# ooowedyn/InkLayer

Hardware: AMD Instinct MI355X
Metric: sketches/sec end-to-end (GroundingDINO+SAM) at 1024x1024 (higher is better)
Workload: dtype f16 (MFMA, f32 accumulate; f32 residual/norm/softmax; split-f16 = fp32-grade operands for patch-embed, neck, mask decoder); 1 GPU; full GroundingDINO Swin-T + SAM ViT-H pipeline, batch=8 per GPU, 1024x1024 synthetic sketches, 16 boxes/sketch, random-init weights; global_batch=8, parallelism=image-parallel x1

## Files before the change

### include/inklayer_hip.h

```cpp
#ifndef INKLAYER_HIP_H
#define INKLAYER_HIP_H

#include <stdint.h>

#ifdef __cplusplus
extern "C" {
#endif

#define INK_ABI_VERSION 10
int ink_abi_version(void);

typedef struct InkGemm {
  const void* A;
  const void* W;
  const float* bias;
  const float* col_scale;
  const float* residual;
  const int32_t* row_map;
  void* C;
  int32_t M, N, K;
  int32_t lda, ldw, ldr, ldc;
  int32_t act;
  int32_t c_f16;
} InkGemm;
// ... 17 lines not shown
int ink_add_f32(const float* a, const float* b, int64_t n_b, float* out, int64_t n, void* stream);

typedef struct InkAttn {
  const void* Q; const void* K; const void* V;
  void* O;
  int64_t ldq, ldk, ldv, ldo;
  int32_t n_batch, n_heads, n_q, n_k, head_dim;
  float scale;
  int32_t bias_mode;
  int32_t grid_w;
  const int32_t* q_batch_rows;
  const int32_t* kv_batch_rows;
  const float* rel_h; const float* rel_w;
  const void* rel_aug;
  const float* dense_bias; const float* dense_mask;
  int32_t n_mask; int32_t rel_f16;
  const int32_t* tok_rows;
  const void* pad_k; const void* pad_v;
} InkAttn;
int ink_flash_attn(const InkAttn* p, void* stream);

int ink_swin_attn(const void* Q, const void* K, const void* V, int64_t ldq, int64_t ldk, int64_t ldv,
                  void* O, int64_t ldo, int32_t n_windows, int32_t n_heads, int32_t ws, float scale,
                  const float* bias_table, const uint8_t* region, int32_t nW, void* stream);

int ink_relpos_bias64_f16(const void* Q, int64_t ldq, const float* rel_pos_h, const float* rel_pos_w, int32_t n_batch,
                          int32_t n_heads, int32_t head_dim, float scale, void* out_h_f16, void* out_w_f16, void* stream);

int ink_relpos_bias(const void* Q, int64_t ldq, const float* rel_pos_h, const float* rel_pos_w,
                    int32_t S, int32_t n_batch, int32_t n_heads, int32_t head_dim, float scale,
                    const int32_t* tok_rows, float* out_h, float* out_w, void* out_aug_f16,
                    void* stream);

int ink_sam_patchify(const void* image_u8, int32_t h, int32_t w, int32_t L, int32_t P,
                     const float* mean3, const float* std3, int32_t chan_reverse, int32_t split,
                     void* out_f16, void* stream);

int ink_resize_u8(const void* src_u8, int32_t h, int32_t w, int32_t channels, void* dst_u8, int32_t oh, int32_t ow,
                  const int32_t* xbounds, const int32_t* xcoef, int32_t kx, const int32_t* ybounds,
                  const int32_t* ycoef, int32_t ky, void* tmp_u8, void* stream);

int ink_im2col3x3_f16(const void* in_f16, int32_t B, int32_t H, int32_t W, int32_t C, int32_t stride, int32_t relu,
                      void* out_f16, void* stream);

int ink_sam_pe_encode(const float* coords01, const float* gauss, int32_t N, int32_t F,
                      const float* add, int32_t n_add, float* out, void* stream);

int ink_sam_prompt_tokens(const float* points, const int32_t* labels, int32_t n_pts, int32_t pad, const float* boxes,
                          const float* gauss, int32_t F, const float* point_emb, const float* not_a_point,
                          const float* out_tok, float input_size, int32_t P, float* out, void* stream);

int ink_sam_mask_embed(const float* mask, const float* emb, const int32_t* emb_rows, const float* params,
                       int32_t n_params, float eps, int32_t P, int32_t g, float* keys, void* split_f16, void* stream);

int ink_sam_mask_logits(const float* up, const float* hyper, int32_t n, int32_t g, int32_t C,
                        float* out, void* stream);

int ink_sam_postprocess(const float* low, int32_t n, int32_t S, int32_t L, int32_t in_h,
                        int32_t in_w, int32_t out_h, int32_t out_w, float thr, void* out_u8,
                        float* out_logits, void* stream);

int ink_ms_deform_attn_forward(const float* value, const int64_t* spatial_shapes_host,
                               const int64_t* level_start_index_host, const float* sampling_loc,
                               const float* attn_weight, int32_t B, int32_t S, int32_t M, int32_t C,
                               int32_t Q, int32_t L, int32_t P, int32_t im2col_step, float* out,
                               void* stream);
// ... 252 lines not shown
```

### inklayer_amd/_lib.py

```python
from __future__ import annotations

import ctypes as C
import os
from pathlib import Path

_LIB_PATH = Path(__file__).resolve().parent / "lib" / "libinklayer_hip.so"
_lib = None

c_void_p, c_int, c_i64, c_float = C.c_void_p, C.c_int32, C.c_int64, C.c_float


class InkGemm(C.Structure):
    _fields_ = [
        ("A", c_void_p), ("W", c_void_p), ("bias", c_void_p), ("col_scale", c_void_p),
        ("residual", c_void_p), ("row_map", c_void_p), ("C", c_void_p),
        ("M", c_int), ("N", c_int), ("K", c_int),
        ("lda", c_int), ("ldw", c_int), ("ldr", c_int), ("ldc", c_int),
        ("act", c_int), ("c_f16", c_int),
    ]


class InkAttn(C.Structure):
    _fields_ = [
        ("Q", c_void_p), ("K", c_void_p), ("V", c_void_p), ("O", c_void_p),
        ("ldq", c_i64), ("ldk", c_i64), ("ldv", c_i64), ("ldo", c_i64),
        ("n_batch", c_int), ("n_heads", c_int), ("n_q", c_int), ("n_k", c_int),
        ("head_dim", c_int), ("scale", c_float), ("bias_mode", c_int), ("grid_w", c_int),
        ("q_batch_rows", c_void_p), ("kv_batch_rows", c_void_p),
        ("rel_h", c_void_p), ("rel_w", c_void_p), ("rel_aug", c_void_p),
        ("dense_bias", c_void_p), ("dense_mask", c_void_p), ("n_mask", c_int), ("rel_f16", c_int),
        ("tok_rows", c_void_p), ("pad_k", c_void_p), ("pad_v", c_void_p),
    ]


SIGNATURES = {
    "ink_abi_version": [],
    "ink_gemm_f16": [C.POINTER(InkGemm), c_void_p],
    "ink_gemm_set_variant": [c_int],
    "ink_gemm_query_variant": [c_int, c_int, c_int],
    "ink_layernorm_rows": [c_void_p, c_i64, c_void_p, c_void_p, c_float, c_void_p, c_int, c_int,
                           c_void_p, c_void_p, c_i64, c_int, c_int, c_void_p, c_i64, c_void_p, c_int, c_void_p],
    "ink_add_split_f16": [c_void_p, c_void_p, c_i64, c_void_p, c_i64, c_int, c_void_p],
    "ink_add_cvt_f16": [c_void_p, c_void_p, c_i64, c_void_p, c_i64, c_void_p],
    "ink_add_f32": [c_void_p, c_void_p, c_i64, c_void_p, c_i64, c_void_p],
    "ink_flash_attn": [C.POINTER(InkAttn), c_void_p],
    "ink_swin_attn": [c_void_p, c_void_p, c_void_p, c_i64, c_i64, c_i64, c_void_p, c_i64, c_int, c_int, c_int, c_float,
                      c_void_p, c_void_p, c_int, c_void_p],
    "ink_sam_patchify": [c_void_p, c_int, c_int, c_int, c_int, C.POINTER(c_float), C.POINTER(c_float),
                         c_int, c_int, c_void_p, c_void_p],
    "ink_im2col3x3_f16": [c_void_p, c_int, c_int, c_int, c_int, c_int, c_int, c_void_p, c_void_p],
    "ink_resize_u8": [c_void_p, c_int, c_int, c_int, c_void_p, c_int, c_int, c_void_p, c_void_p, c_int,
                      c_void_p, c_void_p, c_int, c_void_p, c_void_p],
    "ink_sam_pe_encode": [c_void_p, c_void_p, c_int, c_int, c_void_p, c_int, c_void_p, c_void_p],
    "ink_sam_mask_logits": [c_void_p, c_void_p, c_int, c_int, c_int, c_void_p, c_void_p],
    "ink_sam_prompt_tokens": [c_void_p, c_void_p, c_int, c_int, c_void_p, c_void_p, c_int, c_void_p, c_void_p,
                              c_void_p, c_float, c_int, c_void_p, c_void_p],
    "ink_sam_mask_embed": [c_void_p, c_void_p, c_void_p, c_void_p, c_int, c_float, c_int, c_int, c_void_p, c_void_p,
                           c_void_p],
    "ink_sam_postprocess": [c_void_p, c_int, c_int, c_int, c_int, c_int, c_int, c_int, c_float,
                            c_void_p, c_void_p, c_void_p],
    "ink_sam_amg_stats": [c_void_p, c_int, c_void_p, c_int, c_void_p, c_int, c_int, c_int, c_int, c_int, c_int, C.c_double,
                          C.c_double, c_int, c_int, c_int, c_int, c_void_p, c_void_p, c_void_p, c_void_p],
    "ink_mask_rle_counts": [c_void_p, c_void_p, c_int, c_int, c_int, c_void_p, c_void_p],
    "ink_mask_rle_write": [c_void_p, c_void_p, c_int, c_int, c_int, c_void_p, c_void_p, c_void_p],
    "ink_mask_small_regions_workspace_ints": [c_int, c_int, c_int, C.POINTER(c_i64)],
    "ink_mask_small_regions": [c_void_p, c_int, c_int, c_int, c_int, c_int, c_void_p, c_void_p, c_void_p, c_void_p,
                               c_void_p],
    "ink_box_nms": [c_void_p, c_void_p, c_int, c_float, c_void_p, c_void_p, c_void_p, c_void_p],
    "ink_ms_deform_attn_forward": [c_void_p, C.POINTER(c_i64), C.POINTER(c_i64), c_void_p, c_void_p, c_int,
                                   c_int, c_int, c_int, c_int, c_int, c_int, c_int, c_void_p, c_void_p],
# ... 141 lines not shown
```

### inklayer_amd/csrc/gemm.hip

```cpp
#include <stdlib.h>

#include "mfma_util.h"
#include "../../include/inklayer_hip.h"

namespace {

template <int BK> struct Swz;
template <> struct Swz<64> {
  static __device__ __forceinline__ int f(int row) { return row & 7; }
};
template <> struct Swz<32> {
  static __device__ __forceinline__ int f(int row) { return (-(row >> 2)) & 3; }
};

__device__ __forceinline__ bool residual_preloaded(const InkGemm& p) {
  return p.residual && p.act == INK_ACT_NONE && !p.col_scale;
}

template <int TM>
__device__ __forceinline__ void wave_rows(int (&rows)[TM], const InkGemm& p, int mw, int lane) {
#pragma unroll
  for (int ti = 0; ti < TM; ++ti) {
    const int m = mw + ti * 16 + (lane & 15);
    int r = -1;
    if (m < p.M) r = p.row_map ? p.row_map[m] : m;
    rows[ti] = r;
  }
}

template <int TM, int TN>
__device__ __forceinline__ void init_wave_tile(f32x4 (&acc)[TM][TN], const InkGemm& p, const int (&rows)[TM], int nw,
                                               int lane) {
  const int fq = lane >> 4;
  const bool pre = residual_preloaded(p);
#pragma unroll
  for (int ti = 0; ti < TM; ++ti) {
    const int r = pre ? rows[ti] : -1;
    const float* rp = p.residual + (size_t)max(r, 0) * p.ldr + nw + fq * 4;
#pragma unroll
    for (int j = 0; j < TN; ++j) {
      acc[ti][j] = (f32x4){0.f, 0.f, 0.f, 0.f};
      if (r >= 0 && nw + j * 16 + fq * 4 < p.N) acc[ti][j] = *(const f32x4*)(rp + j * 16);
    }
  }
}

template <int TM, int TN>
__device__ __forceinline__ void add_bias_wave_tile(f32x4 (&acc)[TM][TN], const InkGemm& p, int nw, int lane) {
  const int fq = lane >> 4;
#pragma unroll
  for (int j = 0; j < TN; ++j) {
    const int n = nw + j * 16 + fq * 4;
    f32x4 bv = (f32x4){0.f, 0.f, 0.f, 0.f};
    if (p.bias && n < p.N) bv = *(const f32x4*)(p.bias + n);
#pragma unroll
    for (int ti = 0; ti < TM; ++ti) acc[ti][j] += bv;
  }
}

template <int TM, int TN, int OUT, int MODE = -1>
__device__ __forceinline__ void store_wave_tile(f32x4 (&acc)[TM][TN], const InkGemm& p, char* er,
                                                const int (&rows)[TM], int nw, int lane) {
  constexpr bool F16O = OUT == 1;
  constexpr int WNC = TN * 16, EP = WNC * 4 + 16;
  constexpr int ES = OUT == 0 ? 4 : 8;
  constexpr int CPRW = WNC / ES;
  constexpr int NIT = (16 * CPRW + 63) / 64;
  const int fr = lane & 15, fq = lane >> 4;
  const bool wide16 = OUT != 0 && (p.ldc % 8 == 0);
  const bool res_late = MODE < 0 && p.residual && !residual_preloaded(p);
  const int act = MODE < 0 ? p.act : MODE;
  const bool scaled = MODE < 0 && p.col_scale != nullptr;
  int row_of[NIT], n_of[NIT];
#pragma unroll
  for (int it = 0; it < NIT; ++it) {
    const int c = it * 64 + lane;
    row_of[it] = c < 16 * CPRW ? c / CPRW : 16;
    n_of[it] = nw + (c % CPRW) * ES;
  }

  add_bias_wave_tile<TM, TN>(acc, p, nw, lane);

#pragma unroll
  for (int ti = 0; ti < TM; ++ti) {
#pragma unroll
    for (int j = 0; j < TN; ++j) {
      f32x4 v = acc[ti][j];
      if (act == INK_ACT_GELU) {
#pragma unroll
        for (int r = 0; r < 4; ++r) v[r] = gelu_erf(v[r]);
      } else if (act == INK_ACT_RELU) {
#pragma unroll
        for (int r = 0; r < 4; ++r) v[r] = fmaxf(v[r], 0.f);
      }
      if (scaled) {
        const int n = nw + j * 16 + fq * 4;
        if (n < p.N) v *= *(const f32x4*)(p.col_scale + n);
      }
      if (F16O) {
        *(f16x4*)(er + fr * EP + (j * 16 + fq * 4) * 2) = (f16x4){(f16)v[0], (f16)v[1], (f16)v[2], (f16)v[3]};
      } else {
        *(f32x4*)(er + fr * EP + (j * 16 + fq * 4) * 4) = v;
      }
    }
#pragma unroll
    for (int it = 0; it < NIT; ++it) {
      int r = __builtin_amdgcn_ds_bpermute((row_of[it] & 15) << 2, rows[ti]);
      if (row_of[it] >= 16 || n_of[it] >= p.N) r = -1;
      if (r >= 0) {
        const int c_n = n_of[it];
        const char* src = er + row_of[it] * EP + (c_n - nw) * (F16O ? 2 : 4);
        if (F16O) {
          f16x8 d = *(const f16x8*)src;
          f16* dst = (f16*)p.C + (size_t)r * p.ldc + c_n;
          if (res_late) {
            const float* rp = p.residual + (size_t)r * p.ldr + c_n;
#pragma unroll
            for (int e = 0; e < 8; ++e)
              if (c_n + e < p.N) d[e] = (f16)((float)d[e] + rp[e]);
          }
          if (wide16 && c_n + 8 <= p.N) {
            *(f16x8*)dst = d;
          } else {
            *(f16x4*)dst = (f16x4){d[0], d[1], d[2], d[3]};
            if (c_n + 8 <= p.N) *(f16x4*)(dst + 4) = (f16x4){d[4], d[5], d[6], d[7]};
          }
        } else {
          f32x4 d = *(const f32x4*)src;
          if (res_late) d += *(const f32x4*)(p.residual + (size_t)r * p.ldr + c_n);
          *(f32x4*)((float*)p.C + (size_t)r * p.ldc + c_n) = d;
        }
      }
    }
  }
}

__device__ __forceinline__ void tile_of(int id, int ntm, int ntn, int group_m, int& mt, int& nt) {
  if (group_m > 1) {
    const int per = group_m * ntn;
    const int first = (id / per) * group_m;
    const int gsz = min(ntm - first, group_m);
    mt = first + (id % per) % gsz;
    nt = (id % per) / gsz;
  } else {
    mt = id / ntn;
    nt = id % ntn;
  }
}

constexpr int NS = 2;
template <int BM, int BN, int BK, int WM, int WN>
__global__ __launch_bounds__(WM * WN * 64) void gemm_f16_nt(InkGemm p, int group_m) {
  constexpr int NT = WM * WN * 64;
  constexpr int CPR = BK / 8;
  constexpr int ROWB = BK * 2;
  constexpr int TILE_A = BM * ROWB, TILE_W = BN * ROWB;
  constexpr int STAGE = TILE_A + TILE_W;
  constexpr int IT_A = (BM * CPR) / NT, IT_W = (BN * CPR) / NT;
  constexpr int TM = BM / WM / 16, TN = BN / WN / 16;
  static_assert((BM * CPR) % NT == 0 && (BN * CPR) % NT == 0, "tile/threads mismatch");
  extern __shared__ __attribute__((aligned(16))) char smem[];

  const int tid = threadIdx.x;
  const int lane = tid & 63;
  const int wave = tid >> 6;
  const int wm = wave / WN, wn = wave % WN;

// ... 58 lines not shown
      for (int i0 = 0; i0 < TM; i0 += AG) {
#pragma unroll
        for (int i = 0; i < AG; ++i) a[i] = *(const f16x8*)(bA + offA + (i0 + i) * 16 * ROWB + co);
#pragma unroll
        for (int i = 0; i < AG; ++i)
#pragma unroll
          for (int j = 0; j < TN; ++j)
            acc[i0 + i][j] = __builtin_amdgcn_mfma_f32_16x16x32_f16(w[j], a[i], acc[i0 + i][j], 0, 0, 0);
      }
    }
  };

  stage(0, 0);
  init_wave_tile<TM, TN>(acc, p, rows, n0 + wn * (BN / WN), lane);
  for (int kt = 0; kt < nk; ++kt) {
    asm volatile("s_waitcnt vmcnt(0)" ::: "memory");
    __syncthreads();
    if (kt + 1 < nk) stage((kt + 1) & 1, kt + 1);
    compute(kt & 1);
  }

  constexpr int WNC = BN / WN;
  constexpr int EP = WNC * 4 + 16;
  static_assert(WM * WN * 16 * EP <= NS * STAGE, "epilogue patch must fit in the staging LDS");
  __syncthreads();
  char* er = smem + wave * (16 * EP);
  if (p.c_f16 == 1) {
    store_wave_tile<TM, TN, 1>(acc, p, er, rows, n0 + wn * WNC, lane);
  } else {
    store_wave_tile<TM, TN, 0>(acc, p, er, rows, n0 + wn * WNC, lane);
  }
}

constexpr int PP_RING = 4, PP_TN = 5;
__global__ __launch_bounds__(512) void gemm_f16_nt_pp(InkGemm p, int group_m) {
  constexpr int RING = PP_RING, TN = PP_TN;
  constexpr int BM = 256, BN = 64 * TN, BK = 32, NT = 512;
  constexpr int CPR = BK / 8, ROWB = BK * 2;
  constexpr int TILE_A = BM * ROWB, TILE_W = BN * ROWB, GRAN = TILE_A + TILE_W;
  constexpr int IT_A = (BM * CPR) / NT, IT_W = (BN * CPR) / NT;
  constexpr bool W_TAIL = (BN * CPR) % NT != 0;
  static_assert(!W_TAIL || (BN * CPR) % NT == NT / 2, "tail is exactly the first four waves");
  constexpr int LOADS = IT_A + IT_W;
  constexpr int TM = 8, WNC = 16 * TN;
  constexpr int AHEAD = RING - 2;
  constexpr int AG = 4;
  constexpr int EP = WNC * 4 + 16;
  static_assert(8 * 16 * EP <= RING * GRAN, "patch fits");
  extern __shared__ __attribute__((aligned(16))) char smem[];
  const int tid = threadIdx.x, lane = tid & 63;
  const int wave = __builtin_amdgcn_readfirstlane(tid >> 6);
  const int grp = wave >> 2, wn = wave & 3;
  const int fr = lane & 15, fq = lane >> 4;

  const int ntn = (p.N + BN - 1) / BN, ntm = (p.M + BM - 1) / BM;
  int mt, nt;
  tile_of(xcd_remap(blockIdx.x, ntm * ntn), ntm, ntn, group_m, mt, nt);
  const int m0 = mt * BM, n0 = nt * BN;
  const int G = p.K / BK;
  const f16* __restrict__ A = (const f16*)p.A;
  const f16* __restrict__ W = (const f16*)p.W;
  const f16* srcA[IT_A];
  const f16* srcW[IT_W + (W_TAIL ? 1 : 0)];
#pragma unroll
  for (int it = 0; it < IT_A; ++it) {
    const int pch = it * NT + tid, row = pch / CPR, lch = (pch % CPR) ^ Swz<BK>::f(row);
    srcA[it] = A + (size_t)min(m0 + row, p.M - 1) * p.lda + lch * 8;
  }
#pragma unroll
  for (int it = 0; it < IT_W + (W_TAIL ? 1 : 0); ++it) {
    const int pch = it * NT + tid, row = min(pch / CPR, BN - 1), lch = (pch % CPR) ^ Swz<BK>::f(row);
    srcW[it] = W + (size_t)min(n0 + row, p.N - 1) * p.ldw + lch * 8;
  }
  auto dma = [&](int g, int slot) {
    char* base = smem + slot * GRAN;
#pragma unroll
    for (int it = 0; it < IT_A; ++it)
      __builtin_amdgcn_global_load_lds((gptr_t)(srcA[it] + g * BK), (lptr_t)(base + (it * NT + wave * 64) * 16), 16, 0, 0);
#pragma unroll
    for (int it = 0; it < IT_W; ++it)
      __builtin_amdgcn_global_load_lds((gptr_t)(srcW[it] + g * BK), (lptr_t)(base + TILE_A + (it * NT + wave * 64) * 16), 16, 0, 0);
    if (W_TAIL && grp == 0)
      __builtin_amdgcn_global_load_lds((gptr_t)(srcW[IT_W] + g * BK), (lptr_t)(base + TILE_A + (IT_W * NT + wave * 64) * 16), 16, 0, 0);
  };
  auto wait_ahead = [&]() {
    if (W_TAIL && grp == 0) {
      asm volatile("s_waitcnt vmcnt(%0)" ::"n"((AHEAD - 1) * (LOADS + 1)) : "memory");
    } else {
      asm volatile("s_waitcnt vmcnt(%0)" ::"n"((AHEAD - 1) * LOADS) : "memory");
    }
  };
  auto slot_end = [&]() {
    __builtin_amdgcn_sched_barrier(0);
    __builtin_amdgcn_s_barrier();
    __builtin_amdgcn_sched_barrier(0);
  };

  int rows[TM];
  wave_rows<TM>(rows, p, m0 + grp * 128, lane);
#pragma unroll
  for (int g = 0; g < AHEAD; ++g) dma(g, g);
  f32x4 acc[TM][TN];
  init_wave_tile<TM, TN>(acc, p, rows, n0 + wn * WNC, lane);
  if (residual_preloaded(p)) {
    asm volatile("s_waitcnt vmcnt(0)" ::: "memory");
  } else {
    wait_ahead();
  }
  slot_end();
  if (grp == 1) slot_end();

  const int offA = (grp * 128 + fr) * ROWB;
  const int offW = (wn * WNC + fr) * ROWB;
  const int co = (fq ^ Swz<BK>::f(fr)) << 4;
  f16x8 a[AG], w[TN];
  int cslot = 0, islot = AHEAD % RING;
  auto iter = [&](int g) __attribute__((always_inline)) {
    const char* bA = smem + cslot * GRAN;
    const char* bW = bA + TILE_A;
#pragma unroll
    for (int i = 0; i < AG; ++i) a[i] = *(const f16x8*)(bA + offA + i * 16 * ROWB + co);
#pragma unroll
    for (int j = 0; j < TN; ++j) w[j] = *(const f16x8*)(bW + offW + j * 16 * ROWB + co);
    if (g + AHEAD < G) {
      dma(g + AHEAD, islot);
      wait_ahead();
    } else {
      asm volatile("s_waitcnt vmcnt(0)" ::: "memory");
    }
    slot_end();
    asm volatile("s_waitcnt lgkmcnt(0)" ::: "memory");
    __builtin_amdgcn_sched_barrier(0);
    __builtin_amdgcn_s_setprio(1);
#pragma unroll
    for (int i0 = 0; i0 < TM; i0 += AG) {
#pragma unroll
      for (int i = 0; i < AG; ++i) {
#pragma unroll
        for (int j = 0; j < TN; ++j)
          acc[i0 + i][j] = __builtin_amdgcn_mfma_f32_16x16x32_f16(w[j], a[i], acc[i0 + i][j], 0, 0, 0);
        if (i0 + AG < TM) {
          a[i] = *(const f16x8*)(bA + offA + (i0 + AG + i) * 16 * ROWB + co);
          __builtin_amdgcn_sched_barrier(0);
        }
      }
    }
    __builtin_amdgcn_s_setprio(0);
    slot_end();
    cslot = (cslot + 1 == RING) ? 0 : cslot + 1;
    islot = (islot + 1 == RING) ? 0 : islot + 1;
  };
  for (int g = 0; g < G; ++g) iter(g);
  if (grp == 0) slot_end();

  char* er = smem + wave * (16 * EP);
  const bool plain = !p.col_scale && !(p.residual && !residual_preloaded(p));
  if (p.c_f16) {
    if (plain && p.act == INK_ACT_GELU) {
      store_wave_tile<TM, TN, 1, INK_ACT_GELU>(acc, p, er, rows, n0 + wn * WNC, lane);
    } else if (plain && p.act == INK_ACT_NONE) {
      store_wave_tile<TM, TN, 1, INK_ACT_NONE>(acc, p, er, rows, n0 + wn * WNC, lane);
    } else {
      store_wave_tile<TM, TN, 1>(acc, p, er, rows, n0 + wn * WNC, lane);
    }
  } else {
    if (plain && p.act == INK_ACT_NONE) {
      store_wave_tile<TM, TN, 0, INK_ACT_NONE>(acc, p, er, rows, n0 + wn * WNC, lane);
    } else {
      store_wave_tile<TM, TN, 0>(acc, p, er, rows, n0 + wn * WNC, lane);
    }
  }
}

static int launch_gemm_pp(const InkGemm& p, hipStream_t s, int group_m) {
  if (p.K / 32 < PP_RING) return INK_ERR_ARG;
  constexpr int BN = 64 * PP_TN;
  constexpr int lds = PP_RING * (256 + BN) * 32 * 2;
  static_assert(lds <= 160 * 1024, "LDS budget");
  ink_dyn_lds<gemm_f16_nt_pp>(lds);
  const int ntiles = ((p.M + 255) / 256) * ((p.N + BN - 1) / BN);
  hipLaunchKernelGGL(gemm_f16_nt_pp, dim3(ntiles), dim3(512), lds, s, p, group_m);
  return ink_launch_status();
}

template <int BM, int BN, int BK, int WM, int WN>
static int launch_gemm(const InkGemm& p, hipStream_t s, int group_m = 1) {
  constexpr int lds = NS * (BM + BN) * BK * 2;
  static_assert(lds <= 160 * 1024, "LDS budget");
  ink_dyn_lds<gemm_f16_nt<BM, BN, BK, WM, WN>>(lds);
  const int ntm = (p.M + BM - 1) / BM, ntn = (p.N + BN - 1) / BN;
  hipLaunchKernelGGL((gemm_f16_nt<BM, BN, BK, WM, WN>), dim3(ntm * ntn), dim3(WM * WN * 64), lds, s, p, group_m);
  return ink_launch_status();
}

struct ConvGeom {
  int H, W, C, OH, OW, stride;
};
__device__ __attribute__((aligned(128))) const uint32_t g_conv_zero_row[32] = {};

template <int BK, bool RELU_IN>
__global__ __launch_bounds__(256) void conv3x3_f16_nt(InkGemm p, ConvGeom g) {
  constexpr int BM = 128, BN = 128, WM = 2, WN = 2;
  constexpr int NT = WM * WN * 64;
  constexpr int CPR = BK / 8;
  constexpr int ROWB = BK * 2;
  constexpr int TILE_A = BM * ROWB, TILE_W = BN * ROWB;
  constexpr int STAGE = TILE_A + TILE_W;
  constexpr int IT_A = (BM * CPR) / NT, IT_W = (BN * CPR) / NT;
  constexpr int TM = BM / WM / 16, TN = BN / WN / 16;
  extern __shared__ __attribute__((aligned(16))) char smem[];

  const int tid = threadIdx.x;
  const int lane = tid & 63;
  const int wave = tid >> 6;
// ... 165 lines not shown
  const long tiles256 = (long)((M + 255) / 256) * ((N + 255) / 256);
  const bool n_fits = (N % 256 == 0) || N >= 1024;
  return (tiles256 >= 200 && n_fits) ? 10 : 0;
}
extern "C" int ink_abi_version(void) { return INK_ABI_VERSION; }
extern "C" int ink_gemm_set_variant(int32_t v) {
  INK_CHECK_ARG(v == -1 || v == 0 || v == 10 || v == 45);
  g_variant = v;
  return INK_OK;
}

extern "C" int ink_gemm_f16(const InkGemm* pp, void* stream) {
  INK_CHECK_ARG(pp != nullptr);
  const InkGemm& p = *pp;
  INK_CHECK_ARG(p.A && p.W && p.C);
  INK_CHECK_ARG(p.M > 0 && p.N > 0 && p.K > 0);
  INK_CHECK_ARG(p.K % 32 == 0 && p.N % 4 == 0);
  INK_CHECK_ARG(p.lda % 8 == 0 && p.ldw % 8 == 0 && p.lda >= p.K && p.ldw >= p.K);
  INK_CHECK_ARG(p.ldc % 4 == 0 && p.ldc >= p.N);
  INK_CHECK_ARG(!p.residual || (p.ldr % 4 == 0 && p.ldr >= p.N));
  INK_CHECK_ARG(ink_aligned<16>(p.A, p.W, p.C));
  INK_CHECK_ARG(p.act >= 0 && p.act <= 2);
  INK_CHECK_ARG(p.c_f16 == 0 || p.c_f16 == 1);
  hipStream_t s = (hipStream_t)stream;
  if (p.K % 64 != 0) return launch_gemm<128, 128, 32, 2, 2>(p, s);
  int v = g_variant;
  if (v < 0) v = ink_gemm_query_variant(p.M, p.N, p.K);
  switch (v) {
    case 10: return launch_gemm<256, 256, 64, 4, 4>(p, s, 4);
    case 45: return launch_gemm_pp(p, s, 4);
    default: return launch_gemm<128, 128, 64, 2, 2>(p, s);
  }
}
```

### inklayer_amd/ops.py

```python
from __future__ import annotations

import ctypes as C
from typing import Optional, Sequence, Tuple

import torch

from . import _lib
from ._lib import InkAttn, InkGemm, check

ACT = {None: 0, "none": 0, "gelu": 1, "relu": 2}
F16, F32 = torch.float16, torch.float32


_GEMM_TRACE = None


def set_gemm_trace(lst) -> None:
    global _GEMM_TRACE
    _GEMM_TRACE = lst


_ATTN_TRACE = None


def set_attn_trace(lst) -> None:
    global _ATTN_TRACE
    _ATTN_TRACE = lst


def tracing_off() -> bool:
    return _GEMM_TRACE is None and _ATTN_TRACE is None


_raw_stream = getattr(torch._C, "_cuda_getCurrentRawStream", None)
_cur_device = getattr(torch._C, "_cuda_getDevice", None)


def _stream() -> int:
    if _raw_stream is not None and _cur_device is not None:
        return _raw_stream(_cur_device())
    return torch.cuda.current_stream().cuda_stream


def own_f32(t: torch.Tensor, dev) -> torch.Tensor:
    t = t.detach().to(dev, F32).contiguous()
    if t.untyped_storage().nbytes() > t.numel() * t.element_size():
        t = t.clone()
    return t


def _p(t: Optional[torch.Tensor]) -> Optional[int]:
    if t is None:
        return None
    assert t.is_cuda, "InkLayer HIP ops need GPU tensors (no CPU fallback)"
    return t.data_ptr()


def gemm(a: torch.Tensor, w: torch.Tensor, bias: Optional[torch.Tensor] = None, *,
         act: Optional[str] = None, residual: Optional[torch.Tensor] = None,
         col_scale: Optional[torch.Tensor] = None, row_map: Optional[torch.Tensor] = None,
         out: Optional[torch.Tensor] = None, out_dtype: torch.dtype = F32,
         out_rows: Optional[int] = None) -> torch.Tensor:
    assert a.dtype == F16 and w.dtype == F16
    assert a.dim() == 2 and w.dim() == 2 and a.stride(1) == 1 and w.stride(1) == 1
    M, K = a.shape
    N = w.shape[0]
    assert w.shape[1] == K
    p = InkGemm()
    if out is None:
        rows = out_rows if out_rows is not None else M
        out = torch.empty((rows, N), device=a.device, dtype=out_dtype)
    assert out.dim() == 2 and out.stride(1) == 1 and out.shape[1] == N
    p.A, p.W, p.C = a.data_ptr(), w.data_ptr(), out.data_ptr()
    p.bias, p.col_scale = _p(bias), _p(col_scale)
    p.residual, p.row_map = _p(residual), _p(row_map)
    if bias is not None:
        assert bias.dtype == F32 and bias.numel() == N
    if col_scale is not None:
        assert col_scale.dtype == F32 and col_scale.numel() == N
    if residual is not None:
        assert residual.dtype == F32 and residual.stride(1) == 1 and residual.shape[1] == N
        p.ldr = residual.stride(0)
    if row_map is not None:
        assert row_map.dtype == torch.int32 and row_map.numel() == M
    p.M, p.N, p.K = M, N, K
    p.lda, p.ldw, p.ldc = a.stride(0), w.stride(0), out.stride(0)
    p.act = ACT[act]
    p.c_f16 = 1 if out.dtype == F16 else 0
    assert out.dtype in (F16, F32)
    if _GEMM_TRACE is None:
        check(_lib.lib().ink_gemm_f16(C.byref(p), _stream()), "ink_gemm_f16")
    else:
        e0, e1 = torch.cuda.Event(enable_timing=True), torch.cuda.Event(enable_timing=True)
        e0.record()
        check(_lib.lib().ink_gemm_f16(C.byref(p), _stream()), "ink_gemm_f16")
        e1.record()
        _GEMM_TRACE.append((2.0 * M * N * K, e0, e1, (M, N, K, act or '-', 'res' if residual is not None else '-',
                                                      'map' if row_map is not None else '-', 'f16' if p.c_f16 else 'f32')))
    return out


def layernorm_rows(x: torch.Tensor, gamma: Optional[torch.Tensor], beta: Optional[torch.Tensor],
                   eps: float, *, gather: Optional[torch.Tensor] = None,
                   out_dtype: torch.dtype = F16, out: Optional[torch.Tensor] = None,
                   out2: Optional[torch.Tensor] = None, act: Optional[str] = None,
                   split: bool = False, add: Optional[torch.Tensor] = None,
                   add_batch_rows: Optional[torch.Tensor] = None, rows_per_batch: int = 0,
                   split_f32: Optional[torch.Tensor] = None) -> torch.Tensor:
    assert x.dtype == F32 and x.dim() == 2 and x.stride(1) == 1
    Cdim = x.shape[1]
    rows = gather.numel() if gather is not None else x.shape[0]
    wcols = 3 * Cdim if split else Cdim
    if split:
        assert out_dtype == F16 and out2 is None
    if out is None:
        out = torch.empty((rows, wcols), device=x.device, dtype=out_dtype)
    assert out.shape == (rows, wcols) and out.stride(1) == 1
    oh = out.data_ptr() if out.dtype == F16 else None
    of = out.data_ptr() if out.dtype == F32 else None
    if out2 is not None:
        assert out2.shape == out.shape and out2.stride(0) == out.stride(0) and out2.dtype != out.dtype
        if out2.dtype == F16:
            oh = out2.data_ptr()
        else:
            of = out2.data_ptr()
    if split_f32 is not None:
        assert split and out.stride(0) == 3 * Cdim and split_f32.dtype == F32 and split_f32.is_contiguous()
        assert tuple(split_f32.shape) == (rows, Cdim)
# ... 1327 lines not shown
```

### inklayer_amd/sam.py

```python
from __future__ import annotations

import math
from dataclasses import dataclass, replace
from typing import Dict, List, Optional, Sequence, Tuple

import numpy as np
import torch

from . import ops
from ._lru import LRU

F16, F32 = torch.float16, torch.float32


@dataclass
class SamConfig:
    embed_dim: int = 1280
    depth: int = 32
    num_heads: int = 16
    global_attn_indexes: Tuple[int, ...] = (7, 15, 23, 31)
    window_size: int = 14
    img_size: int = 1024
    patch_size: int = 16
    mlp_ratio: float = 4.0
# ... 197 lines not shown
            "the fused decoder kernels (csrc/proj_ln.hip, csrc/upscale_tail.hip) are built for SAM's widths"
        self.scale = cfg.head_dim ** -0.5
        sd = state_dict
        dev = self.dev

        def h(name):
            return sd[name].detach().to(torch.float32).to(dev, F16).contiguous()

        def f(name):
            return ops.own_f32(sd[name], dev)

        def ws(name, shape=None):
            t = sd[name].detach().to(dev, torch.float32)
            return ops.split_weight(t if shape is None else shape(t))

        self.w: Dict[str, torch.Tensor] = {}
        w = self.w
        P = cfg.patch_size
        w["pe.ws"] = ws("image_encoder.patch_embed.proj.weight", lambda t: t.reshape(D, 3 * P * P))
        w["pe.b"] = f("image_encoder.patch_embed.proj.bias")
        w["pos"] = f("image_encoder.pos_embed").reshape(self.T, D).contiguous()
        for i in range(cfg.depth):
            p = f"image_encoder.blocks.{i}."
            for n in ("norm1.weight", "norm1.bias", "norm2.weight", "norm2.bias", "attn.qkv.bias",
                      "attn.proj.bias", "mlp.lin1.bias", "mlp.lin2.bias", "attn.rel_pos_h",
                      "attn.rel_pos_w"):
                w[f"b{i}.{n}"] = f(p + n)
            for n in ("attn.qkv.weight", "attn.proj.weight", "mlp.lin1.weight", "mlp.lin2.weight"):
                w[f"b{i}.{n}"] = h(p + n)
            if i not in cfg.global_attn_indexes:
                qb = w[f"b{i}.attn.qkv.bias"]
                w[f"b{i}.pad_k"] = qb[D:2 * D].to(F16).contiguous()
                w[f"b{i}.pad_v"] = qb[2 * D:].to(F16).contiguous()
        w["neck0.ws"] = ws("image_encoder.neck.0.weight", lambda t: t.reshape(E, D))
        w["neck1.w"], w["neck1.b"] = f("image_encoder.neck.1.weight"), f("image_encoder.neck.1.bias")
        w["neck2.ws"] = ws("image_encoder.neck.2.weight", lambda t: t.permute(0, 2, 3, 1).reshape(E, 9, E)) \
            .reshape(E, 27 * E).contiguous()
        w["neck3.w"], w["neck3.b"] = f("image_encoder.neck.3.weight"), f("image_encoder.neck.3.bias")

        w["gauss"] = f("prompt_encoder.pe_layer.positional_encoding_gaussian_matrix")
        w["no_mask"] = f("prompt_encoder.no_mask_embed.weight").reshape(-1).contiguous()
        w["pt_emb"] = torch.cat([f(f"prompt_encoder.point_embeddings.{i}.weight") for i in range(4)], 0).contiguous()
        if "prompt_encoder.not_a_point_embed.weight" in sd:
            w["not_a_point"] = f("prompt_encoder.not_a_point_embed.weight").reshape(-1).contiguous()
        md = "prompt_encoder.mask_downscaling."
        md_names = ("0.weight", "0.bias", "1.weight", "1.bias", "3.weight", "3.bias", "4.weight", "4.bias", "6.weight",
                    "6.bias")
        if all(md + n in sd for n in md_names):
            w["mask_ds"] = torch.cat([sd[md + n].detach().to(torch.float32).reshape(-1) for n in md_names]) \
                .to(dev).contiguous()
        ar = (torch.arange(g, dtype=torch.float32) + 0.5) / g
        grid_xy = torch.stack([ar[None, :].expand(g, g), ar[:, None].expand(g, g)], -1).reshape(-1, 2)
        self.dense_pe = ops.sam_pe_encode(grid_xy.contiguous().to(dev), w["gauss"])

        t = "mask_decoder.transformer."
        def attn(dst, src):
            for n in ("q_proj", "k_proj", "v_proj", "out_proj"):
                w[f"{dst}.{n}.ws"] = ws(f"{src}.{n}.weight")
                w[f"{dst}.{n}.b"] = f(f"{src}.{n}.bias")

        def cat(dst, names):
            for sfx in (".ws", ".b"):
                w[dst + sfx] = torch.cat([w[n + sfx] for n in names]).contiguous()

        pe_split = ops.add_split_f16(self.dense_pe)
        for i in range(cfg.dec_depth):
# ... 95 lines not shown
            ops.sam_patchify(img, cfg.img_size, cfg.patch_size, cfg.pixel_mean, cfg.pixel_std,
                             chan_reverse, self.buf_patches[b * T:(b + 1) * T], split=True)
        ops.gemm(self.buf_patches[:B * T], w["pe.ws"], w["pe.b"], residual=self.pos_rep[:B * T], out=x)
        if upto is None and self.graph_blocks and ops.tracing_off():
            return self._blocks_graphed(B)
        return self._blocks(B, upto)

    graph_blocks = False
    graph_cache_size = 2

    def _blocks_graphed(self, B: int) -> torch.Tensor:
        g = self._enc_graphs.get(B)
        if g is None:
            self._enc_seen[B] = self._enc_seen.get(B, 0) + 1
            if self._enc_seen[B] < 2:
                return self._blocks(B, None)
            x0 = self.x[:B * self.T].clone()
            cur = torch.cuda.current_stream(self.dev)
            side = torch.cuda.Stream(device=self.dev)
            side.wait_stream(cur)
            with torch.cuda.stream(side):
                self._blocks(B, None)
                self.x[:B * self.T].copy_(x0)
            cur.wait_stream(side)
            graph = torch.cuda.CUDAGraph()
            with torch.cuda.graph(graph):
                out = self._blocks(B, None)
            self.x[:B * self.T].copy_(x0)
            g = (graph, out)
            self._enc_graphs.put(B, g)
        g[0].replay()
        return g[1].clone()

    def _blocks(self, B: int, upto: Optional[int]) -> torch.Tensor:
        cfg, w, T, D = self.cfg, self.w, self.T, self.cfg.embed_dim
        H, Mw = cfg.num_heads, self.Mw
        x = self.x[:B * T]
        nblk = cfg.depth if upto is None else upto
        calib = getattr(self, "_calib", None)
        for i in range(nblk):
            k = f"b{i}."
            y = ops.layernorm_rows(x, w[k + "norm1.weight"], w[k + "norm1.bias"], 1e-6, out=self.y[:B * T])
            if calib is not None:
                calib[k + "attn.qkv"] = y.float().mean(0)
            qkv = ops.gemm(y, w[k + "attn.qkv.weight"], w[k + "attn.qkv.bias"], out=self.qkv[:B * T])
            q, kk, v = qkv[:, :D], qkv[:, D:2 * D], qkv[:, 2 * D:]
            if i in cfg.global_attn_indexes:
                rh, rw = ops.relpos_bias(q, w[k + "attn.rel_pos_h"], w[k + "attn.rel_pos_w"], S=cfg.grid,
                                         n_batch=B, n_heads=H, head_dim=cfg.head_dim, scale=self.scale,
                                         out=(self.rel_h, self.rel_w), f16_tables=self.rel_f16)
                o = ops.flash_attn(q, kk, v, n_batch=B, n_heads=H, head_dim=cfg.head_dim, scale=self.scale,
                                   rel_h=rh, rel_w=rw, grid_w=cfg.grid, out=self.att[:B * T])
            else:
                wm = self.win_map[:B * Mw]
                nb = B * self.nwin * self.nwin
                aug = ops.relpos_bias(q, w[k + "attn.rel_pos_h"], w[k + "attn.rel_pos_w"],
                                      S=cfg.window_size, n_batch=nb, n_heads=H, head_dim=cfg.head_dim,
                                      scale=self.scale, out=self.rel_aug, tok_rows=wm)
                o = ops.flash_attn(q, kk, v, n_batch=nb, n_heads=H, head_dim=cfg.head_dim, scale=self.scale,
                                   n_q=cfg.window_size ** 2, n_k=cfg.window_size ** 2,
                                   rel_aug=aug, grid_w=cfg.window_size, tok_rows=wm,
                                   pad_k=w[k + "pad_k"], pad_v=w[k + "pad_v"], out=self.att[:B * T])
            if calib is not None:
                calib[k + "attn.proj"] = o.float().mean(0)
            ops.gemm(o, w[k + "attn.proj.weight"], w[k + "attn.proj.bias"], residual=x, out=x)
            y = ops.layernorm_rows(x, w[k + "norm2.weight"], w[k + "norm2.bias"], 1e-6, out=self.y[:B * T])
            hd = ops.gemm(y, w[k + "mlp.lin1.weight"], w[k + "mlp.lin1.bias"], act="gelu", out=self.hid[:B * T])
            if calib is not None:
                calib[k + "mlp.lin1"], calib[k + "mlp.lin2"] = y.float().mean(0), hd.float().mean(0)
            ops.gemm(hd, w[k + "mlp.lin2.weight"], w[k + "mlp.lin2.bias"], residual=x, out=x)
        if upto is not None:
            return x.view(B, T, D)
        n0 = ops.gemm(ops.add_split_f16(x), w["neck0.ws"])
        n1 = ops.layernorm_rows(n0, w["neck1.w"], w["neck1.b"], 1e-6, split=True)
        n2 = ops.gemm(ops.im2col3x3(n1, B, cfg.grid, cfg.grid), w["neck2.ws"])
        emb = ops.layernorm_rows(n2, w["neck3.w"], w["neck3.b"], 1e-6, out_dtype=F32)
        return emb.view(B, T, cfg.prompt_embed_dim)

    def decode(self, emb: torch.Tensor, boxes_input_frame: np.ndarray | torch.Tensor,
               input_hw: Tuple[int, int], orig_hw: Tuple[int, int], want_logits: bool = False):
        boxes = torch.as_tensor(np.asarray(boxes_input_frame), dtype=torch.float32).reshape(-1, 4)
        low, iou = self.decode_low_res(emb.reshape(1, self.T, -1), boxes, [0] * boxes.shape[0])
        res = ops.sam_postprocess(low, self.cfg.img_size, input_hw, orig_hw, self.cfg.mask_threshold, want_logits)
        if want_logits:
            return res[0], low, iou, res[1]
        return res

    def decode_low_res(self, emb: torch.Tensor, boxes: torch.Tensor, img_of_box: Sequence[int]):
        low, iou = self.decode_prompts(emb, img_of_box, boxes=boxes)
        return low.view(low.shape[0], *low.shape[-2:]), iou

# ... 250 lines not shown
```

Before: 117.9 sketches/s.

## Fuse windowed rel-pos bias computation into SAM QKV GEMM epilogue

Adds a templated variant of the pipelined f16 GEMM that, for the Q-column tiles of windowed attention blocks, computes the decomposed relative-position bias (q · rel_pos_h/w) with MFMA directly from the freshly produced Q values. It writes the f16 augmented bias rows into the rel_aug buffer. The relpos table is preloaded into extra LDS, and scratch reuses the drained ring buffer. This removes a separate relpos_bias kernel launch and its re-read of Q for the 28 windowed SAM blocks, at the cost of more epilogue work and LDS in the QKV GEMM.

```diff
diff --git a/include/inklayer_hip.h b/include/inklayer_hip.h
--- a/include/inklayer_hip.h
+++ b/include/inklayer_hip.h
@@ -73,6 +73,14 @@
                     const int32_t* tok_rows, float* out_h, float* out_w, void* out_aug_f16,
                     void* stream);
 
+typedef struct InkQkvRelpos {
+  const void* tab_f16;
+  void* out_aug;
+  float inv_scale;
+  int32_t grid, window, n_heads, head_dim;
+} InkQkvRelpos;
+int ink_gemm_f16_qkv_relpos(const InkGemm* p, const InkQkvRelpos* r, void* stream);
+
 int ink_sam_patchify(const void* image_u8, int32_t h, int32_t w, int32_t L, int32_t P,
                      const float* mean3, const float* std3, int32_t chan_reverse, int32_t split,
                      void* out_f16, void* stream);
diff --git a/inklayer_amd/_lib.py b/inklayer_amd/_lib.py
--- a/inklayer_amd/_lib.py
+++ b/inklayer_amd/_lib.py
@@ -17,6 +17,13 @@
         ("M", c_int), ("N", c_int), ("K", c_int),
         ("lda", c_int), ("ldw", c_int), ("ldr", c_int), ("ldc", c_int),
         ("act", c_int), ("c_f16", c_int),
+    ]
+
+
+class InkQkvRelpos(C.Structure):
+    _fields_ = [
+        ("tab_f16", c_void_p), ("out_aug", c_void_p), ("inv_scale", c_float),
+        ("grid", c_int), ("window", c_int), ("n_heads", c_int), ("head_dim", c_int),
     ]
 
 
@@ -36,6 +43,7 @@
 SIGNATURES = {
     "ink_abi_version": [],
     "ink_gemm_f16": [C.POINTER(InkGemm), c_void_p],
+    "ink_gemm_f16_qkv_relpos": [C.POINTER(InkGemm), C.POINTER(InkQkvRelpos), c_void_p],
     "ink_gemm_set_variant": [c_int],
     "ink_gemm_query_variant": [c_int, c_int, c_int],
     "ink_layernorm_rows": [c_void_p, c_i64, c_void_p, c_void_p, c_float, c_void_p, c_int, c_int,
diff --git a/inklayer_amd/csrc/gemm.hip b/inklayer_amd/csrc/gemm.hip
--- a/inklayer_amd/csrc/gemm.hip
+++ b/inklayer_amd/csrc/gemm.hip
@@ -45,6 +45,63 @@
   }
 }
 
+struct QkvAug {
+  const char* tab;
+  char* sc;
+  f16* out;
+  float inv_scale;
+  int grid, nwin, n_heads, head;
+  uint32_t mg2, mg;
+};
+constexpr int AUG_S = 14, AUG_TROW = 160, AUG_SROW = 80;
+
+__device__ __forceinline__ f16x8 cat4(const f16x4& a, const f16x4& b) {
+  return (f16x8){a[0], a[1], a[2], a[3], b[0], b[1], b[2], b[3]};
+}
+
+template <int TM>
+__device__ __forceinline__ void relpos_wave_tile(const QkvAug& g, const f16x4 (&qh)[TM][5], const int (&rows)[TM], int lane) {
+  constexpr int S = AUG_S;
+  const int fr = lane & 15, fq = lane >> 4;
+  const f16x4 z4 = {0, 0, 0, 0};
+  f16x8 tf[4][3];
+#pragma unroll
+  for (int t = 0; t < 4; ++t) {
+    const char* tr = g.tab + (t * 16 + fr) * AUG_TROW + fq * 8;
+#pragma unroll
+    for (int s = 0; s < 3; ++s) tf[t][s] = cat4(*(const f16x4*)(tr + s * 64), s < 2 ? *(const f16x4*)(tr + s * 64 + 32) : z4);
+  }
+  char* const row = g.sc + fr * AUG_SROW;
+  if (fq == 0) *(f16x4*)(row + 56) = z4;
+  const int tok = lane >> 2;
+#pragma unroll
+  for (int ti = 0; ti < TM; ++ti) {
+    const int m = rows[ti];
+    const uint32_t mu = (uint32_t)max(m, 0);
+    const uint32_t b = __umulhi(mu, g.mg2), rem = mu - __umul24(b, g.grid * g.grid);
+    const uint32_t y = __umulhi(rem, g.mg), x = rem - __umul24(y, g.grid);
+    const uint32_t wy = __umul24(y, 1171) >> 14, wx = __umul24(x, 1171) >> 14;
+    const int qy = (int)(y - __umul24(wy, S)), qx = (int)(x - __umul24(wx, S));
+    const uint32_t win = __umul24(b, g.nwin * g.nwin) + __umul24(wy, g.nwin) + wx;
+    const int arow = m < 0 ? -1 : (int)(__umul24(__umul24(win, g.n_heads) + g.head, S * S) + __umul24(qy, S) + qx);
+#pragma unroll
+    for (int t = 0; t < 4; ++t) {
+      f32x4 d = (f32x4){0.f, 0.f, 0.f, 0.f};
+#pragma unroll
+      for (int s = 0; s < 3; ++s)
+        d = __builtin_amdgcn_mfma_f32_16x16x32_f16(tf[t][s], cat4(qh[ti][2 * s], s < 2 ? qh[ti][2 * s + 1] : z4), d, 0, 0, 0);
+      const int base = (t >= 2 ? qx : qy) + S - 1 - ((t & 1) * 16 + 4 * fq);
+#pragma unroll
+      for (int r = 0; r < 4; ++r) {
+        const int j = base - r;
+        if (j >= 0 && j < S) *(f16*)(row + ((t >= 2 ? S : 0) + j) * 2) = (f16)(d[r] * g.inv_scale);
+      }
+    }
+    const int r = __builtin_amdgcn_ds_bpermute(tok << 2, arow);
+    if (r >= 0) *(f16x8*)(g.out + (int64_t)r * 32 + (lane & 3) * 8) = *(const f16x8*)(g.sc + tok * AUG_SROW + (lane & 3) * 16);
+  }
+}
+
 template <int TM, int TN>
 __device__ __forceinline__ void add_bias_wave_tile(f32x4 (&acc)[TM][TN], const InkGemm& p, int nw, int lane) {
   const int fq = lane >> 4;
@@ -58,9 +115,9 @@
   }
 }
 
-template <int TM, int TN, int OUT, int MODE = -1>
+template <int TM, int TN, int OUT, int MODE = -1, bool AUG = false>
 __device__ __forceinline__ void store_wave_tile(f32x4 (&acc)[TM][TN], const InkGemm& p, char* er,
-                                                const int (&rows)[TM], int nw, int lane) {
+                                                const int (&rows)[TM], int nw, int lane, const QkvAug& ag = QkvAug{}) {
   constexpr bool F16O = OUT == 1;
   constexpr int WNC = TN * 16, EP = WNC * 4 + 16;
   constexpr int ES = OUT == 0 ? 4 : 8;
@@ -80,6 +137,8 @@
   }
 
   add_bias_wave_tile<TM, TN>(acc, p, nw, lane);
+  static_assert(!AUG || (OUT == 1 && TN == 5), "AUG: one head of 80 f16 per wave tile row");
+  f16x4 qh[AUG ? TM : 1][AUG ? TN : 1];
 
 #pragma unroll
   for (int ti = 0; ti < TM; ++ti) {
@@ -98,7 +157,9 @@
         if (n < p.N) v *= *(const f32x4*)(p.col_scale + n);
       }
       if (F16O) {
-        *(f16x4*)(er + fr * EP + (j * 16 + fq * 4) * 2) = (f16x4){(f16)v[0], (f16)v[1], (f16)v[2], (f16)v[3]};
+        const f16x4 h = {(f16)v[0], (f16)v[1], (f16)v[2], (f16)v[3]};
+        *(f16x4*)(er + fr * EP + (j * 16 + fq * 4) * 2) = h;
+        if constexpr (AUG) qh[ti][j] = h;
       } else {
         *(f32x4*)(er + fr * EP + (j * 16 + fq * 4) * 4) = v;
       }
@@ -133,6 +194,7 @@
       }
     }
   }
+  if constexpr (AUG) relpos_wave_tile<TM>(ag, qh, rows, lane);
 }
 
 __device__ __forceinline__ void tile_of(int id, int ntm, int ntn, int group_m, int& mt, int& nt) {
@@ -257,8 +319,18 @@
   }
 }
 
+struct RelposArgs {
+  const f16* tab;
+  f16* out_aug;
+  float inv_scale;
+  int grid, nwin, n_heads;
+  uint32_t mg2, mg;
+};
 constexpr int PP_RING = 4, PP_TN = 5;
-__global__ __launch_bounds__(512) void gemm_f16_nt_pp(InkGemm p, int group_m) {
+template <class... RP>
+__global__ __launch_bounds__(512) void gemm_f16_nt_pp(InkGemm p, int group_m, RP... rpa) {
+  constexpr bool RELPOS = sizeof...(RP) == 1;
+  static_assert(sizeof...(RP) <= 1 && (std::is_same_v<RP, RelposArgs> && ...), "at most one RelposArgs");
   constexpr int RING = PP_RING, TN = PP_TN;
   constexpr int BM = 256, BN = 64 * TN, BK = 32, NT = 512;
   constexpr int CPR = BK / 8, ROWB = BK * 2;
@@ -323,6 +395,15 @@
 
   int rows[TM];
   wave_rows<TM>(rows, p, m0 + grp * 128, lane);
+  if constexpr (RELPOS) {
+    const RelposArgs& rp = (rpa, ...);
+    if (nt < rp.n_heads / 4) {
+      const f16* src = rp.tab + (wave * 64 + lane) * 8;
+      char* dst = smem + RING * GRAN + wave * 64 * 16;
+      __builtin_amdgcn_global_load_lds((gptr_t)src, (lptr_t)dst, 16, 0, 0);
+      if (wave < 2) __builtin_amdgcn_global_load_lds((gptr_t)(src + NT * 8), (lptr_t)(dst + NT * 16), 16, 0, 0);
+    }
+  }
 #pragma unroll
   for (int g = 0; g < AHEAD; ++g) dma(g, g);
   f32x4 acc[TM][TN];
@@ -379,6 +460,19 @@
   if (grp == 0) slot_end();
 
   char* er = smem + wave * (16 * EP);
+  if constexpr (RELPOS) {
+    const RelposArgs& rp = (rpa, ...);
+    if (nt < rp.n_heads / 4) {
+      constexpr int SC0 = 8 * 16 * EP;
+      static_assert(SC0 + 8 * 16 * AUG_SROW <= RING * GRAN && SC0 % 16 == 0, "fits the drained ring");
+      const QkvAug ag = {smem + RING * GRAN, smem + SC0 + wave * (16 * AUG_SROW), rp.out_aug, rp.inv_scale, rp.grid,
+                         rp.nwin, rp.n_heads, nt * 4 + wn, rp.mg2, rp.mg};
+      store_wave_tile<TM, TN, 1, INK_ACT_NONE, true>(acc, p, er, rows, n0 + wn * WNC, lane, ag);
+    } else {
+      store_wave_tile<TM, TN, 1, INK_ACT_NONE>(acc, p, er, rows, n0 + wn * WNC, lane);
+    }
+    return;
+  }
   const bool plain = !p.col_scale && !(p.residual && !residual_preloaded(p));
   if (p.c_f16) {
     if (plain && p.act == INK_ACT_GELU) {
@@ -397,14 +491,21 @@
   }
 }
 
-static int launch_gemm_pp(const InkGemm& p, hipStream_t s, int group_m) {
+static int launch_gemm_pp(const InkGemm& p, hipStream_t s, int group_m, const RelposArgs* rp = nullptr) {
   if (p.K / 32 < PP_RING) return INK_ERR_ARG;
   constexpr int BN = 64 * PP_TN;
   constexpr int lds = PP_RING * (256 + BN) * 32 * 2;
   static_assert(lds <= 160 * 1024, "LDS budget");
-  ink_dyn_lds<gemm_f16_nt_pp>(lds);
   const int ntiles = ((p.M + 255) / 256) * ((p.N + BN - 1) / BN);
-  hipLaunchKernelGGL(gemm_f16_nt_pp, dim3(ntiles), dim3(512), lds, s, p, group_m);
+  if (rp) {
+    constexpr int lds_rp = lds + 64 * AUG_TROW;
+    static_assert(lds_rp <= 160 * 1024, "LDS budget");
+    ink_dyn_lds<gemm_f16_nt_pp<RelposArgs>>(lds_rp);
+    hipLaunchKernelGGL(gemm_f16_nt_pp<RelposArgs>, dim3(ntiles), dim3(512), lds_rp, s, p, group_m, *rp);
+  } else {
+    ink_dyn_lds<gemm_f16_nt_pp<>>(lds);
+    hipLaunchKernelGGL(gemm_f16_nt_pp<>, dim3(ntiles), dim3(512), lds, s, p, group_m);
+  }
   return ink_launch_status();
 }
 
@@ -636,3 +737,24 @@
     default: return launch_gemm<128, 128, 64, 2, 2>(p, s);
   }
 }
+
+extern "C" int ink_gemm_f16_qkv_relpos(const InkGemm* pp, const InkQkvRelpos* rr, void* stream) {
+  INK_CHECK_ARG(pp != nullptr && rr != nullptr);
+  const InkGemm& p = *pp;
+  const InkQkvRelpos& r = *rr;
+  INK_CHECK_ARG(p.A && p.W && p.C && r.tab_f16 && r.out_aug);
+  INK_CHECK_ARG(p.M > 0 && p.N > 0 && p.K > 0);
+  INK_CHECK_ARG(p.K % 32 == 0 && p.K / 32 >= PP_RING);
+  INK_CHECK_ARG(p.lda % 8 == 0 && p.ldw % 8 == 0 && p.lda >= p.K && p.ldw >= p.K);
+  INK_CHECK_ARG(p.ldc % 4 == 0 && p.ldc >= p.N);
+  INK_CHECK_ARG(p.c_f16 == 1 && p.act == INK_ACT_NONE && !p.residual && !p.col_scale && !p.row_map);
+  INK_CHECK_ARG(r.head_dim == 80 && r.n_heads > 0 && r.n_heads % 4 == 0 && p.N == 3 * r.n_heads * 80);
+  INK_CHECK_ARG(r.window == AUG_S && r.grid >= 2 && r.grid <= 1024 && r.inv_scale > 0.f);
+  INK_CHECK_ARG(ink_aligned<16>(p.A, p.W, p.C, p.bias, r.tab_f16, r.out_aug));
+  const int64_t g2 = (int64_t)r.grid * r.grid, nwin = (r.grid + AUG_S - 1) / AUG_S;
+  INK_CHECK_ARG((int64_t)p.M * g2 < (1LL << 32));
+  INK_CHECK_ARG(((p.M + g2 - 1) / g2) * nwin * nwin * r.n_heads * (AUG_S * AUG_S) < INT32_MAX);
+  const RelposArgs a = {(const f16*)r.tab_f16, (f16*)r.out_aug, r.inv_scale, r.grid, (int)nwin, r.n_heads,
+                        (uint32_t)((1ULL << 32) / (uint64_t)g2 + 1), (uint32_t)((1ULL << 32) / (uint64_t)r.grid + 1)};
+  return launch_gemm_pp(p, (hipStream_t)stream, 4, &a);
+}
diff --git a/inklayer_amd/ops.py b/inklayer_amd/ops.py
--- a/inklayer_amd/ops.py
+++ b/inklayer_amd/ops.py
@@ -1,12 +1,12 @@
 from __future__ import annotations
 
 import ctypes as C
-from typing import Optional, Sequence, Tuple
+from typing import NamedTuple, Optional, Sequence, Tuple
 
 import torch
 
 from . import _lib
-from ._lib import InkAttn, InkGemm, check
+from ._lib import InkAttn, InkGemm, InkQkvRelpos, check
 
 ACT = {None: 0, "none": 0, "gelu": 1, "relu": 2}
 F16, F32 = torch.float16, torch.float32
@@ -56,11 +56,28 @@
     return t.data_ptr()
 
 
+class QkvRelpos(NamedTuple):
+    tab: torch.Tensor
+    out_aug: torch.Tensor
+    scale: float
+    grid: int
+    window: int
+    n_heads: int
+    head_dim: int
+
+
+def relpos_table(rel_pos_h: torch.Tensor, rel_pos_w: torch.Tensor) -> torch.Tensor:
+    assert rel_pos_h.shape == rel_pos_w.shape == (27, 80)
+    tab = torch.zeros(64, 80, device=rel_pos_h.device, dtype=F16)
+    tab[:27], tab[32:59] = rel_pos_h.to(F16), rel_pos_w.to(F16)
+    return tab
+
+
 def gemm(a: torch.Tensor, w: torch.Tensor, bias: Optional[torch.Tensor] = None, *,
          act: Optional[str] = None, residual: Optional[torch.Tensor] = None,
          col_scale: Optional[torch.Tensor] = None, row_map: Optional[torch.Tensor] = None,
          out: Optional[torch.Tensor] = None, out_dtype: torch.dtype = F32,
-         out_rows: Optional[int] = None) -> torch.Tensor:
+         out_rows: Optional[int] = None, relpos: Optional[QkvRelpos] = None) -> torch.Tensor:
     assert a.dtype == F16 and w.dtype == F16
     assert a.dim() == 2 and w.dim() == 2 and a.stride(1) == 1 and w.stride(1) == 1
     M, K = a.shape
@@ -88,12 +105,21 @@
     p.act = ACT[act]
     p.c_f16 = 1 if out.dtype == F16 else 0
     assert out.dtype in (F16, F32)
+    if relpos is None:
+        launch = lambda: check(_lib.lib().ink_gemm_f16(C.byref(p), _stream()), "ink_gemm_f16")
+    else:
+        assert relpos.tab.dtype == F16 and relpos.tab.is_contiguous() and tuple(relpos.tab.shape) == (64, 80)
+        assert relpos.out_aug.dtype == F16 and relpos.out_aug.is_cuda and relpos.tab.is_cuda
+        r = InkQkvRelpos(relpos.tab.data_ptr(), relpos.out_aug.data_ptr(), 1.0 / C.c_float(relpos.scale).value, relpos.grid,
+                         relpos.window, relpos.n_heads, relpos.head_dim)
+        launch = lambda: check(_lib.lib().ink_gemm_f16_qkv_relpos(C.byref(p), C.byref(r), _stream()),
+                               "ink_gemm_f16_qkv_relpos")
     if _GEMM_TRACE is None:
-        check(_lib.lib().ink_gemm_f16(C.byref(p), _stream()), "ink_gemm_f16")
+        launch()
     else:
         e0, e1 = torch.cuda.Event(enable_timing=True), torch.cuda.Event(enable_timing=True)
         e0.record()
-        check(_lib.lib().ink_gemm_f16(C.byref(p), _stream()), "ink_gemm_f16")
+        launch()
         e1.record()
         _GEMM_TRACE.append((2.0 * M * N * K, e0, e1, (M, N, K, act or '-', 'res' if residual is not None else '-',
                                                       'map' if row_map is not None else '-', 'f16' if p.c_f16 else 'f32')))
diff --git a/inklayer_amd/sam.py b/inklayer_amd/sam.py
--- a/inklayer_amd/sam.py
+++ b/inklayer_amd/sam.py
@@ -253,6 +253,8 @@
                 qb = w[f"b{i}.attn.qkv.bias"]
                 w[f"b{i}.pad_k"] = qb[D:2 * D].to(F16).contiguous()
                 w[f"b{i}.pad_v"] = qb[2 * D:].to(F16).contiguous()
+                if self._qkv_relpos_ok():
+                    w[f"b{i}.rel_tab"] = ops.relpos_table(w[f"b{i}.attn.rel_pos_h"], w[f"b{i}.attn.rel_pos_w"])
         w["neck0.ws"] = ws("image_encoder.neck.0.weight", lambda t: t.reshape(E, D))
         w["neck1.w"], w["neck1.b"] = f("image_encoder.neck.1.weight"), f("image_encoder.neck.1.bias")
         w["neck2.ws"] = ws("image_encoder.neck.2.weight", lambda t: t.permute(0, 2, 3, 1).reshape(E, 9, E)) \
@@ -414,6 +416,12 @@
         g[0].replay()
         return g[1].clone()
 
+    qkv_relpos = True
+
+    def _qkv_relpos_ok(self) -> bool:
+        cfg = self.cfg
+        return cfg.head_dim == 80 and cfg.num_heads % 4 == 0 and cfg.window_size == 14
+
     def _blocks(self, B: int, upto: Optional[int]) -> torch.Tensor:
         cfg, w, T, D = self.cfg, self.w, self.T, self.cfg.embed_dim
         H, Mw = cfg.num_heads, self.Mw
@@ -425,7 +433,10 @@
             y = ops.layernorm_rows(x, w[k + "norm1.weight"], w[k + "norm1.bias"], 1e-6, out=self.y[:B * T])
             if calib is not None:
                 calib[k + "attn.qkv"] = y.float().mean(0)
-            qkv = ops.gemm(y, w[k + "attn.qkv.weight"], w[k + "attn.qkv.bias"], out=self.qkv[:B * T])
+            fused = (self.qkv_relpos and calib is None and i not in cfg.global_attn_indexes and self._qkv_relpos_ok())
+            rp = ops.QkvRelpos(w[k + "rel_tab"], self.rel_aug, self.scale, cfg.grid, cfg.window_size, H,
+                               cfg.head_dim) if fused else None
+            qkv = ops.gemm(y, w[k + "attn.qkv.weight"], w[k + "attn.qkv.bias"], out=self.qkv[:B * T], relpos=rp)
             q, kk, v = qkv[:, :D], qkv[:, D:2 * D], qkv[:, 2 * D:]
             if i in cfg.global_attn_indexes:
                 rh, rw = ops.relpos_bias(q, w[k + "attn.rel_pos_h"], w[k + "attn.rel_pos_w"], S=cfg.grid,
@@ -436,9 +447,9 @@
             else:
                 wm = self.win_map[:B * Mw]
                 nb = B * self.nwin * self.nwin
-                aug = ops.relpos_bias(q, w[k + "attn.rel_pos_h"], w[k + "attn.rel_pos_w"],
-                                      S=cfg.window_size, n_batch=nb, n_heads=H, head_dim=cfg.head_dim,
-                                      scale=self.scale, out=self.rel_aug, tok_rows=wm)
+                aug = self.rel_aug if fused else ops.relpos_bias(
+                    q, w[k + "attn.rel_pos_h"], w[k + "attn.rel_pos_w"], S=cfg.window_size, n_batch=nb, n_heads=H,
+                    head_dim=cfg.head_dim, scale=self.scale, out=self.rel_aug, tok_rows=wm)
                 o = ops.flash_attn(q, kk, v, n_batch=nb, n_heads=H, head_dim=cfg.head_dim, scale=self.scale,
                                    n_q=cfg.window_size ** 2, n_k=cfg.window_size ** 2,
                                    rel_aug=aug, grid_w=cfg.window_size, tok_rows=wm,
```

After: 119.0 sketches/s (median of 6 runs). About the same (+0.9%).
